# mandt-lab/vbq

Measured on AMD Instinct MI355X. Metric: quantized latents/sec (32-lambda sweep; one count per (element, lambda) pair and entropy-model build), higher is better.
Workload: dtype f32; 1 GPU; kodak24_c256 [36864 x 256] f32, 32-lambda sweep, N=10; step = two-pass entropy-model build (quantizer.py:82-150); elements_per_gpu=9437184, lambdas=32, parallelism=element-sharded x1, launch=one HIP graph replay per step

## Files before the change

### include/vbq.h

```cpp
#ifndef VBQ_H_
#define VBQ_H_

#include <stddef.h>
#include <stdint.h>

#ifdef __cplusplus
extern "C" {
#endif

#define VBQ_ABI_VERSION 5

enum {
    VBQ_OK = 0,
    VBQ_ERR_INVALID_ARGUMENT = -1,
    VBQ_ERR_UNSUPPORTED = -2,
    VBQ_ERR_LAUNCH = -3,
    VBQ_ERR_WORKSPACE = -4
};

enum {
    VBQ_LAYOUT_BC = 0,
    VBQ_LAYOUT_CB = 1,
    VBQ_LAYOUT_BC_TO_CB = 2
};
// ... 3 lines not shown
    VBQ_MODE_F64_SCORE = 1
};

int vbq_abi_version(void);
const char *vbq_last_error(void);


enum { VBQ_GRID_K1 = 0, VBQ_GRID_K1T = 1 };
int vbq_solve_grid(int32_t kernel, int64_t n_rows, int32_t n_ch, int32_t workgroups_per_cu, int32_t reserved_workgroups,
                   int64_t *h_grid);

int vbq_device_count(void);
int vbq_device_name(int dev, char *buf, size_t buflen);

size_t vbq_quantize_workspace_bytes(int32_t n_ch, int32_t n_lambda, int32_t N);

int vbq_check_inputs_f32(const float *d_mu, const float *d_sigma, int64_t n, uint32_t *d_bad, void *stream);

int vbq_quantize_f32(const float *d_mu, const float *d_sigma, int64_t n_rows, int32_t n_ch,
                     int32_t layout, const float *d_table_lm, const float *d_level_len,
                     const double *h_lambdas, int32_t n_lambda, int32_t N, int32_t mode,
                     uint16_t *d_out_idx, float *d_out_zhat, float *d_out_bits,
                     void *d_workspace, size_t workspace_bytes, void *stream);

int vbq_n_bit_intervals_f32(const float *d_z_cb, int64_t n_rows, int32_t n_ch, const float *d_table_lm, int32_t N,
                            float *d_left, float *d_right, void *stream);

int vbq_quantize_rows_f32(const float *d_mu, const float *d_sigma, int64_t n_rows, int32_t n_ch,
                          int32_t layout, const float *d_table_lm, const float *d_level_len,
                          const double *h_lambdas, int32_t n_lambda, int32_t N, int32_t mode,
                          uint16_t *d_out_idx, float *d_out_zhat, float *d_out_bits,
                          void *d_workspace, size_t workspace_bytes, int64_t row_begin, int64_t row_end,
                          int32_t workgroups_per_cu, int32_t reserved_workgroups, void *stream);

int vbq_level_counts_f32(const float *d_mu, const float *d_sigma, int64_t n_rows, int32_t n_ch,
                         int32_t layout, const float *d_table_lm, const float *d_level_len,
                         const double *h_lambdas, int32_t n_lambda, int32_t N, int64_t *d_level_counts,
                         void *d_workspace, size_t workspace_bytes, int32_t reserved_workgroups, void *stream);

int vbq_code_lengths_from_counts(const void *d_counts, int32_t counts_are_i32, int64_t n,
                                 const float *d_lut, int64_t lut_n, int32_t level_period,
                                 float *d_out_len, float *d_out_model, void *stream);

typedef void (*vbq_f32_loop)(char **args, const intptr_t *dimensions, const intptr_t *steps, void *data);
typedef struct vbq_host_stage {
    const void *h_counts;
    int32_t counts_are_i32;
    int32_t add_level;
    int64_t n_rows;
    int64_t K;
    float add_n_smoothing;
    int32_t status;
    vbq_f32_loop log2_loop;
    void *log2_data;
    float *h_out_model;
    float *h_out_len;
    int64_t runs;
} vbq_host_stage;
int vbq_host_neg_log2_freq_f32(const void *h_counts, int32_t counts_are_i32, int64_t n_rows, int64_t K, float add_n_smoothing,
                               int32_t add_level, vbq_f32_loop log2_loop, void *log2_data, float *h_out_model,
                               float *h_out_len);
void vbq_host_stage_run(void *stage);

int vbq_argmax_candidates_f32(const float *d_P, const float *d_len, int32_t len_per_lambda,
                              const float *d_mu, const float *d_sigma, int64_t n_elems,
                              const double *h_lambdas, int32_t n_lambda, int32_t M, int32_t mode,
// ... 163 lines not shown
```

### vbq_amd/_lib.py

```python
from __future__ import annotations

import ctypes as C
import os


_LIB = None

c_f32p = C.c_void_p
c_u16p = C.c_void_p

OK = 0
ABI_VERSION = 5
LAYOUT_BC, LAYOUT_CB, LAYOUT_BC_TO_CB = 0, 1, 2
MODE_F32, MODE_F64_SCORE = 0, 1
BMSHJ_PARAMS_PER_CHANNEL = 43
COMM_ID_BYTES = 128

SIGNATURES = {
    "vbq_abi_version": (C.c_int, []),
    "vbq_last_error": (C.c_char_p, []),
    "vbq_solve_grid": (C.c_int, [C.c_int32, C.c_int64, C.c_int32, C.c_int32, C.c_int32, C.POINTER(C.c_int64)]),
    "vbq_device_count": (C.c_int, []),
    "vbq_device_name": (C.c_int, [C.c_int, C.c_char_p, C.c_size_t]),
    "vbq_quantize_workspace_bytes": (C.c_size_t, [C.c_int32, C.c_int32, C.c_int32]),
    "vbq_check_inputs_f32": (C.c_int, [C.c_void_p, C.c_void_p, C.c_int64, C.c_void_p, C.c_void_p]),
    "vbq_quantize_f32": (C.c_int, [C.c_void_p, C.c_void_p, C.c_int64, C.c_int32, C.c_int32, C.c_void_p, C.c_void_p,
                                   C.POINTER(C.c_double), C.c_int32, C.c_int32, C.c_int32, C.c_void_p, C.c_void_p,
                                   C.c_void_p, C.c_void_p, C.c_size_t, C.c_void_p]),
    "vbq_n_bit_intervals_f32": (C.c_int, [C.c_void_p, C.c_int64, C.c_int32, C.c_void_p, C.c_int32, C.c_void_p, C.c_void_p,
                                          C.c_void_p]),
    "vbq_quantize_rows_f32": (C.c_int, [C.c_void_p, C.c_void_p, C.c_int64, C.c_int32, C.c_int32, C.c_void_p, C.c_void_p,
                                        C.POINTER(C.c_double), C.c_int32, C.c_int32, C.c_int32, C.c_void_p, C.c_void_p,
                                        C.c_void_p, C.c_void_p, C.c_size_t, C.c_int64, C.c_int64, C.c_int32, C.c_int32, C.c_void_p]),
    "vbq_level_counts_f32": (C.c_int, [C.c_void_p, C.c_void_p, C.c_int64, C.c_int32, C.c_int32, C.c_void_p, C.c_void_p,
                                       C.POINTER(C.c_double), C.c_int32, C.c_int32, C.c_void_p, C.c_void_p, C.c_size_t,
                                       C.c_int32, C.c_void_p]),
    "vbq_code_lengths_from_counts": (C.c_int, [C.c_void_p, C.c_int32, C.c_int64, C.c_void_p, C.c_int64, C.c_int32,
                                               C.c_void_p, C.c_void_p, C.c_void_p]),
    "vbq_host_neg_log2_freq_f32": (C.c_int, [C.c_void_p, C.c_int32, C.c_int64, C.c_int64, C.c_float, C.c_int32, C.c_void_p, C.c_void_p,
                                             C.c_void_p, C.c_void_p]),
    "vbq_host_stage_run": (None, [C.c_void_p]),
    "vbq_histogram_rows_u16": (C.c_int, [C.c_void_p, C.c_int64, C.c_int32, C.c_int32, C.c_int32, C.c_int32, C.c_void_p,
                                         C.c_int32, C.c_int64, C.c_int64, C.c_void_p]),
    "vbq_xi_intervals_f64": (C.c_int, [C.c_void_p, C.c_int64, C.c_int32, C.c_void_p, C.c_void_p, C.c_void_p]),
    "vbq_xi_select_f64": (C.c_int, [C.c_void_p, C.c_void_p, C.c_void_p, C.c_int64, C.c_int32, C.c_double, C.c_void_p,
                                    C.c_void_p, C.c_void_p, C.c_void_p, C.c_void_p]),
    "vbq_quantize_notebook_f64": (C.c_int, [C.c_void_p, C.c_void_p, C.c_int64, C.c_void_p, C.POINTER(C.c_double),
                                            C.c_int32, C.c_int32, C.c_void_p, C.c_void_p, C.c_void_p]),
    "vbq_histogram_u16": (C.c_int, [C.c_void_p, C.c_int64, C.c_int32, C.c_int32, C.c_int32, C.c_int32, C.c_void_p,
                                    C.c_void_p]),
    "vbq_histogram_u16_i32": (C.c_int, [C.c_void_p, C.c_int64, C.c_int32, C.c_int32, C.c_int32, C.c_int32,
                                        C.c_void_p, C.c_void_p]),
    "vbq_histogram_models_u16": (C.c_int, [C.c_void_p, C.c_int64, C.c_int32, C.c_int32, C.c_int32, C.c_void_p, C.c_int32,
                                           C.c_void_p, C.c_int64, C.c_void_p, C.c_void_p]),
    "vbq_index_max_u16": (C.c_int, [C.c_void_p, C.c_int64, C.c_void_p, C.c_void_p]),
    "vbq_moments_f32": (C.c_int, [C.c_void_p, C.c_int64, C.c_int32, C.c_int32, C.c_void_p, C.c_void_p]),
    "vbq_numpy_sum_sq_workspace_bytes": (C.c_size_t, [C.c_int64]),
    "vbq_numpy_sum_sq_f32": (C.c_int, [C.c_void_p, C.c_int64, C.c_void_p, C.c_void_p, C.c_size_t, C.c_void_p]),
    "vbq_numpy_row_sums_workspace_bytes": (C.c_size_t, [C.c_int64, C.c_int64]),
    "vbq_numpy_row_sums_f32": (C.c_int, [C.c_void_p, C.c_int64, C.c_int64, C.c_void_p, C.c_void_p, C.c_size_t, C.c_void_p]),
    "vbq_gather_f32": (C.c_int, [C.c_void_p, C.c_int64, C.c_int32, C.c_int32, C.c_int32, C.c_int32, C.c_void_p,
                                 C.c_int32, C.c_void_p, C.c_int32, C.c_void_p]),
    "vbq_rd_sums_u16": (C.c_int, [C.c_void_p, C.c_void_p, C.c_void_p, C.c_int64, C.c_int32, C.c_int32, C.c_int32, C.c_int32,
                                  C.c_void_p, C.c_void_p, C.c_int32, C.c_void_p, C.c_void_p]),
    "vbq_transpose_f32": (C.c_int, [C.c_void_p, C.c_int64, C.c_int64, C.c_void_p, C.c_void_p]),
    "vbq_transpose_planes": (C.c_int, [C.c_void_p, C.c_int64, C.c_int64, C.c_int64, C.c_int32, C.c_void_p, C.c_void_p]),
# ... 121 lines not shown
```

### vbq_amd/csrc/vbq_latents.hip

```cpp
#include <atomic>

#include <type_traits>

#include "vbq_common.h"

namespace vbq {
namespace {

__global__ void __launch_bounds__(256)
k_prep_planes(const float *__restrict__ in0, const float *__restrict__ in1, long rows, long cols, float *__restrict__ out0,
              float *__restrict__ out1, int sqrt1, int v4) {
    __shared__ float tile[64][65];
    const bool second = blockIdx.y == 1;
    const float *in = second ? in1 : in0;
    float *out = second ? out1 : out0;
    const int kind = second ? sqrt1 : 0;
    auto f = [kind](float x) { return kind == 0 ? x : sqrtf(kind == 2 ? expf(x) : x); };
    const long ctiles = (cols + 63) / 64;
    const long r0 = ((long)blockIdx.x / ctiles) * 64, c0 = ((long)blockIdx.x % ctiles) * 64;
    if (v4 && r0 + 64 <= rows && c0 + 64 <= cols) {
        float4 v[4];
#pragma unroll
        for (int k = 0; k < 4; ++k) {
            const int i = threadIdx.x + 256 * k, lr = i >> 4, lc = (i & 15) * 4;
// ... 441 lines not shown
    VBQ_REQUIRE(d_lut_levels && n_lut_levels > n_rows && d_level_counts && d_level_len && d_raw_models && d_counts,
                VBQ_ERR_INVALID_ARGUMENT, "vbq_build_entropy_models_f32: null pointer argument, or a code-length table shorter than n_rows + 1");
    VBQ_REQUIRE((d_models == nullptr) == (d_lut_ranks == nullptr) && (!d_lut_ranks || n_lut_ranks > n_rows), VBQ_ERR_INVALID_ARGUMENT,
                "vbq_build_entropy_models_f32: d_models and d_lut_ranks go together (n_rows + 1 entries)");
    const size_t need = vbq_build_entropy_models_workspace_bytes(n_rows, n_ch, n_lambda, N);
    VBQ_REQUIRE(d_workspace && workspace_bytes >= need, VBQ_ERR_WORKSPACE,
                "vbq_build_entropy_models_f32: workspace of %zu bytes given, %zu needed", workspace_bytes, need);
    VBQ_REQUIRE((reinterpret_cast<uintptr_t>(d_workspace) & 255) == 0, VBQ_ERR_INVALID_ARGUMENT,
                "vbq_build_entropy_models_f32: workspace must be 256-byte aligned");
    const size_t E = (size_t)n_rows * (size_t)n_ch;
    const int64_t N1 = N + 1;
    char *w = static_cast<char *>(d_workspace);
    float *mu_cb = reinterpret_cast<float *>(w);
    w += align256(E * sizeof(float));
    float *sg_cb = reinterpret_cast<float *>(w);
    w += align256(E * sizeof(float));
    uint16_t *idx = reinterpret_cast<uint16_t *>(w);
    w += align256((size_t)n_lambda * E * sizeof(uint16_t));
    const size_t qws = vbq_quantize_workspace_bytes(n_ch, n_lambda, N);
    hipStream_t st = reinterpret_cast<hipStream_t>(stream);
    int rc = vbq_prep_planes_f32(d_means_bc, d_spread_bc, spread_kind, n_rows, n_ch, mu_cb, sg_cb, stream);
    if (rc != VBQ_OK) return rc;
    hipError_t e = hipMemsetAsync(d_level_counts, 0, sizeof(int64_t) * (size_t)n_lambda * (size_t)n_ch * (size_t)N1, st);
    if (e != hipSuccess) {
        set_error("vbq_build_entropy_models_f32: hipMemsetAsync: %s", hipGetErrorString(e));
        return VBQ_ERR_LAUNCH;
    }
    rc = vbq_level_counts_f32(mu_cb, sg_cb, n_rows, n_ch, VBQ_LAYOUT_CB, d_table_lm, nullptr, h_lambdas, n_lambda, N, d_level_counts, w, qws,
                              reserved_workgroups, stream);
    if (rc != VBQ_OK) return rc;
    rc = vbq_code_lengths_from_counts(d_level_counts, 0, (int64_t)n_lambda * n_ch * N1, d_lut_levels, n_lut_levels, (int32_t)N1, d_level_len,
                                      d_raw_models, stream);
    if (rc != VBQ_OK) return rc;
    rc = vbq_quantize_rows_f32(mu_cb, sg_cb, n_rows, n_ch, VBQ_LAYOUT_CB, d_table_lm, d_level_len, h_lambdas, n_lambda, N, VBQ_MODE_F32, idx,
                               nullptr, nullptr, w, qws, 0, n_rows, 0, reserved_workgroups, stream);
    if (rc != VBQ_OK) return rc;
    return vbq_histogram_models_u16(idx, n_rows, n_ch, n_lambda, N, d_counts, counts_are_i32, d_lut_ranks, n_lut_ranks, d_models, stream);
}
```

### vbq_amd/csrc/vbq_quantize_fast.hip

```cpp
#include <string.h>

#include "vbq_common.h"

namespace vbq {
namespace {

constexpr int kFastThreads = 256;
#ifndef VBQ_FAST_NE
#define VBQ_FAST_NE 2
#endif
#ifndef VBQ_FAST_WAVES
#define VBQ_FAST_WAVES 4
#endif
#ifndef VBQ_SLOW_INLINE
#define VBQ_SLOW_INLINE __noinline__
#endif
constexpr int kFastNE = VBQ_FAST_NE;

__device__ __forceinline__ float dist_cost(float P, float mu, double rinv) {
    const float d = __fsub_rn(P, mu);
    const float t = (float)__dmul_rn((double)d, rinv);
    const float q = __fmul_rn(t, t);
    return __fmul_rn(0.5f, q);
}
// ... 73 lines not shown
        const float po = tb[off + jo];
        const float dj = dist_cost(pj, z, sg);
        const float dn = dist_cost(po, z, sg);
        const bool j_is_left = below && !swap;
        r.dL = j_is_left ? dj : dn;
        r.dR = j_is_left ? dn : dj;
        r.posL = j_is_left ? j : (uint32_t)jo;
        r.posR = j_is_left ? (uint32_t)jo : j;
    }
    g = 2 * g + (below ? 1u : 0u);
    return r;
}

template <int N>
__device__ VBQ_SLOW_INLINE uint32_t exact_rank_scan(const float *tb, float z, float sigma, const float *pen) {
    const double sg = __ddiv_rn(1.0, (double)sigma);
    uint32_t g = 0;
    float bestL = 0.f, bestR = 0.f;
    uint32_t rkL = 0, rkR = 0;
    for (int n = 0; n <= N; ++n) {
        const LevelInfo<N> li = descend<N>(tb, n, z, sg, g);
        const float p = pen[n];
        const float cL = __fadd_rn(li.dL, p);
        if (n == 0 || cL < bestL) { bestL = cL; rkL = ((2 * li.posL + 1) << (N - n)) - 1; }
        if (n >= 1) {
            const float cR = __fadd_rn(li.dR, p);
            if (n == 1 || cR < bestR) { bestR = cR; rkR = ((2 * li.posR + 1) << (N - n)) - 1; }
        }
    }
    if (N == 0) return rkL;
    return (bestL <= bestR) ? rkL : rkR;
}

template <int N, int MODE>
__global__ void __launch_bounds__(kFastThreads, VBQ_FAST_WAVES)
k_quant_fast(const float *__restrict__ mu, const float *__restrict__ sg, long n_per_ch, long ch_stride, int C,
             const float *__restrict__ table, Lambdas32 lam, const float *__restrict__ len,
             int L, uint16_t *__restrict__ out_idx, float *__restrict__ out_zhat,
             float *__restrict__ out_bits, long E, int vec_ok, int dbg,
             unsigned long long *__restrict__ level_counts) {
    constexpr int T = table_size(N);
    constexpr int N1 = N + 1;
    constexpr int NE = kFastNE;
    constexpr bool EXTRA = MODE == 1;
    constexpr bool COUNT = MODE == 2;
    const bool never_flag = dbg == 2;
    constexpr int PS = (N1 + 3) & ~3;
    __shared__ float tb[T + 1];
    __shared__ uint32_t scratch[N1 * NE * kFastThreads];
    __shared__ __align__(16) float penl[kMaxLambdaChunk * PS];
    const int c = blockIdx.y;
    if (COUNT) {
        for (int i = threadIdx.x; i < N1 * NE * kFastThreads; i += blockDim.x) scratch[i] = 0;
    }
    for (int i = threadIdx.x; i < T; i += blockDim.x) tb[i] = table[(long)c * T + i];
    int odd = 0;
    for (int i = threadIdx.x; i < L * PS; i += blockDim.x) {
        const int l = i / PS, n = i - l * PS;
        const float p = n < N1 ? __fmul_rn(lam.lam[l], len ? len[((long)l * C + c) * N1 + n] : (float)n) : 0.0f;
        penl[i] = p;
        odd |= (len != nullptr && !(p == 0.0f || (p >= 1.8189894e-12f && p <= 1.1805916e21f))) ? 1 : 0;
    }
    const bool force_slow = dbg == 1 || __syncthreads_or(odd) != 0;

    const long base = (long)c * ch_stride;
    const long nquads = (n_per_ch + NE - 1) / NE;

    auto load_group = [&](long q, float (&m)[NE], float (&sv)[NE]) {
        const long i0 = q * NE;
        if (!(vec_ok & 2) && (vec_ok & 1) && (i0 + NE <= n_per_ch)) {
            if constexpr (NE == 4) {
                const float4 mv = *reinterpret_cast<const float4 *>(mu + base + i0);
                const float4 s4v = *reinterpret_cast<const float4 *>(sg + base + i0);
                m[0] = mv.x; m[1] = mv.y; m[2] = mv.z; m[3] = mv.w;
                sv[0] = s4v.x; sv[1] = s4v.y; sv[2] = s4v.z; sv[3] = s4v.w;
            } else {
                const float2 mv = *reinterpret_cast<const float2 *>(mu + base + i0);
                const float2 s2v = *reinterpret_cast<const float2 *>(sg + base + i0);
// ... 120 lines not shown
                            lvl[k] = (uint32_t)N - (uint32_t)__builtin_ctz(exact_rank_scan<N>(tb, m4[k], s4[k], pp) + 1u);
                }
                const uint32_t lane = threadIdx.x & 63u;
                const uint32_t inc = (lane & 16u) ? 0x10000u : 1u;
#pragma unroll
                for (int k = 0; k < NE; ++k)
                    if (i0 + k < n_per_ch) atomicAdd(&scratch[((uint32_t)(l * N1) + lvl[k]) * 16u + (lane & 15u)], inc);
                continue;
            }
            uint32_t pk[NE];
#pragma unroll
            for (int k = 0; k < NE; ++k) {
                const int n1 = __builtin_ctz(~ne[k]);
                pk[k] = scratch[(n1 * NE + k) * kFastThreads + threadIdx.x];
            }
            uint64_t fm[NE];
#pragma unroll
            for (int k = 0; k < NE; ++k) {
                const uint64_t multi = __builtin_amdgcn_uicmp((uint32_t)__popc(ne[k]), (uint32_t)N, 33);
                const uint32_t thr = __float_as_uint(__fmul_rn(S[k], 1.9073486328125e-06f));
                const uint64_t lr_close = __builtin_amdgcn_uicmp(pk[k], thr, 37);
                rank[k] = pk[k] & ((2u << N) - 1u);
                fm[k] = never_flag ? 0ull : (force_slow ? ~0ull : (multi | lr_close));
            }
            uint64_t any_flag = 0;
#pragma unroll
            for (int k = 0; k < NE; ++k) any_flag |= fm[k];
            if (any_flag != 0) {
                const uint32_t lane = __lane_id();
#pragma unroll
                for (int k = 0; k < NE; ++k)
                    if ((fm[k] >> lane) & 1ull) rank[k] = exact_rank_scan<N>(tb, m4[k], s4[k], pp);
            }
            const long o = (long)l * E + base + i0;
            float zh[NE], bt[NE];
            if (EXTRA) {
#pragma unroll
                for (int k = 0; k < NE; ++k) {
                    const uint32_t kk = rank[k] + 1;
                    const int tz = __builtin_ctz(kk);
                    const int lvl = N - tz;
                    const uint32_t pos = kk >> (tz + 1);
                    zh[k] = tb[(1 << lvl) - 1 + pos];
                    bt[k] = len ? len[((long)l * C + c) * N1 + lvl] : (float)lvl;
                }
            }
            if (full) {
                if constexpr (NE == 4) {
                    uint2 pk2;
                    pk2.x = rank[0] | (rank[1] << 16);
                    pk2.y = rank[2] | (rank[3] << 16);
                    *reinterpret_cast<uint2 *>(out_idx + o) = pk2;
                    if (EXTRA) {
                        if (out_zhat) *reinterpret_cast<float4 *>(out_zhat + o) = make_float4(zh[0], zh[1], zh[2], zh[3]);
                        if (out_bits) *reinterpret_cast<float4 *>(out_bits + o) = make_float4(bt[0], bt[1], bt[2], bt[3]);
                    }
                } else {
                    store_idx2<false>(reinterpret_cast<uint32_t *>(out_idx + o), rank[0] | (rank[1] << 16));
                    if (EXTRA) {
                        if (out_zhat) *reinterpret_cast<float2 *>(out_zhat + o) = make_float2(zh[0], zh[1]);
                        if (out_bits) *reinterpret_cast<float2 *>(out_bits + o) = make_float2(bt[0], bt[1]);
                    }
                }
            } else {
#pragma unroll
                for (int k = 0; k < NE; ++k) {
                    if (i0 + k < n_per_ch) {
                        out_idx[o + k] = (uint16_t)rank[k];
                        if (EXTRA) {
                            if (out_zhat) out_zhat[o + k] = zh[k];
                            if (out_bits) out_bits[o + k] = bt[k];
                        }
                    }
                }
            }
        }
    }
    if constexpr (COUNT) {
        __syncthreads();
        for (int i = threadIdx.x; i < L * N1; i += blockDim.x) {
            unsigned int v = 0;
#pragma unroll
            for (int j = 0; j < 16; ++j) {
                const unsigned int w = scratch[i * 16 + j];
                v += (w & 0xffffu) + (w >> 16);
            }
            const int l = i / N1, n = i - l * N1;
            if (v) atomicAdd(&level_counts[((long)l * C + c) * N1 + n], (unsigned long long)v);
        }
    }
}


#ifndef VBQ_HULL_WAVES
#define VBQ_HULL_WAVES 4
#endif
#ifndef VBQ_HULL_NE
#define VBQ_HULL_NE 2
#endif
#ifndef VBQ_HULL_THREADS
#define VBQ_HULL_THREADS 256
#endif
constexpr int kHullThreads = VBQ_HULL_THREADS;
#ifndef VBQ_HULL_COPIES
#define VBQ_HULL_COPIES 16
#endif
constexpr int kHullKeys = 2048;
// ... 831 lines not shown
        }
        constexpr int64_t max_iters = 65000 / ((64 / 32) * (kFastThreads / 64) * kFastNE);
        if (counting && (iters + gx - 1) / gx > max_iters) gx = (iters + max_iters - 1) / max_iters;
    }
    if (gx < 1) gx = 1;
    *out_gx = gx;
    *out_resident = resident;
}

template <int N>
int launch_quant_fast(const float *mu, const float *sg, int64_t n_per_ch, int64_t ch_stride, int32_t n_ch, const float *table,
                      const Lambdas32 &lam, const float *len, int32_t L, uint16_t *out_idx, float *out_zhat,
                      float *out_bits, int64_t E, int vec_ok,
                      unsigned long long *level_counts, int wg_per_cu, int reserved, hipStream_t st) {
    int64_t gx = 1;
    bool resident = false;
    quant_fast_grid(n_per_ch, n_ch, wg_per_cu, reserved, level_counts != nullptr, &gx, &resident);
    if (resident) vec_ok |= 4;
    const dim3 grid((unsigned)gx, (unsigned)n_ch), block(kFastThreads);
    const int dbg = fast_debug();
    if (level_counts)
        hipLaunchKernelGGL((k_quant_fast<N, 2>), grid, block, 0, st, mu, sg, (long)n_per_ch, (long)ch_stride, (int)n_ch, table,
                           lam, len, (int)L, out_idx, out_zhat, out_bits, (long)E, vec_ok, dbg, level_counts);
    else if (out_zhat || out_bits)
        hipLaunchKernelGGL((k_quant_fast<N, 1>), grid, block, 0, st, mu, sg, (long)n_per_ch, (long)ch_stride, (int)n_ch, table,
                           lam, len, (int)L, out_idx, out_zhat, out_bits, (long)E, vec_ok, dbg, level_counts);
    else
        hipLaunchKernelGGL((k_quant_fast<N, 0>), grid, block, 0, st, mu, sg, (long)n_per_ch, (long)ch_stride, (int)n_ch, table,
                           lam, len, (int)L, out_idx, out_zhat, out_bits, (long)E, vec_ok, dbg, level_counts);
    VBQ_CHECK_LAUNCH("quant_fast");
    return VBQ_OK;
}

template <int N>
int launch_quant_pruned(const float *mu, const float *sg, int64_t n_per_ch, int64_t ch_stride, int32_t n_ch, const float *table,
                        const Lambdas32 &lam, const float *len, int32_t L, uint16_t *out_idx, int64_t E, int vec_ok, hipStream_t st) {
    if (L < 1 || L > kPrunedMaxL) return 1;
    const int64_t npairs = (n_per_ch + 1) / 2;
    int64_t gx = (npairs + 255) / 256;
    int64_t cap = (int64_t)num_cus() * 4 / n_ch;
    if (cap < 1) cap = 1;
    if (gx > cap) gx = cap;
    const int dbg = fast_debug();
    const dim3 grid((unsigned)gx, (unsigned)n_ch), block(256);
#define VBQ_PRUNED_CASE(LLv)                                                                                          \
    case LLv:                                                                                                          \
        hipLaunchKernelGGL((k_quant_pruned<N, LLv>), grid, block, 0, st, mu, sg, (long)n_per_ch, (long)ch_stride, (int)n_ch, \
                           table, lam, len, out_idx, (long)E, vec_ok, dbg);                                            \
        break;
    switch (L) {
        VBQ_PRUNED_CASE(1) VBQ_PRUNED_CASE(2) VBQ_PRUNED_CASE(3) VBQ_PRUNED_CASE(4)
        default: return 1;
    }
#undef VBQ_PRUNED_CASE
    VBQ_CHECK_LAUNCH("quant_pruned");
    return VBQ_OK;
}


static bool build_hull_sweep(const double *lam, int L, HullSweep &sw) {
    if (L < 1 || L > 32) return false;
    int order[32];
    for (int i = 0; i < L; ++i) order[i] = i;
    for (int i = 1; i < L; ++i)
        for (int j = i; j > 0 && (float)lam[order[j]] < (float)lam[order[j - 1]]; --j) { const int t = order[j]; order[j] = order[j - 1]; order[j - 1] = t; }
    int prev_key = -1;
// ... 96 lines not shown
                                       const Lambdas32 &, const float *, int32_t, uint16_t *, float *, float *, int64_t, \
                                       int, unsigned long long *, int, int, hipStream_t);
VBQ_FOR_EACH_N(VBQ_INST_FAST)
#undef VBQ_INST_FAST
#define VBQ_INST_PRUNED(NN)                                                                                           \
    template int launch_quant_pruned<NN>(const float *, const float *, int64_t, int64_t, int32_t, const float *,     \
                                         const Lambdas32 &, const float *, int32_t, uint16_t *, int64_t, int, hipStream_t);
VBQ_FOR_EACH_N(VBQ_INST_PRUNED)
#undef VBQ_INST_PRUNED

}

extern "C" int vbq_solve_grid(int32_t kernel, int64_t n_rows, int32_t n_ch, int32_t workgroups_per_cu, int32_t reserved_workgroups,
                              int64_t *h_grid) {
    using namespace vbq;
    VBQ_REQUIRE(h_grid && n_rows >= 1 && n_ch >= 1 && n_ch <= 65535, VBQ_ERR_INVALID_ARGUMENT, "vbq_solve_grid: bad sizes or null pointer");
    VBQ_REQUIRE(kernel == VBQ_GRID_K1 || kernel == VBQ_GRID_K1T, VBQ_ERR_INVALID_ARGUMENT, "vbq_solve_grid: unknown kernel %d", kernel);
    VBQ_REQUIRE(workgroups_per_cu >= 0 && workgroups_per_cu <= 5, VBQ_ERR_INVALID_ARGUMENT, "vbq_solve_grid: workgroups_per_cu=%d not in 0..5",
                workgroups_per_cu);
    const int reserved = reserved_workgroups < 0 ? 0 : reserved_workgroups;
    if (kernel == VBQ_GRID_K1) {
        int64_t gx = 1;
        bool resident = false;
        quant_fast_grid(n_rows, n_ch, workgroups_per_cu, reserved, false, &gx, &resident);
        h_grid[0] = gx;
        h_grid[2] = resident ? 1 : 0;
    } else {
        h_grid[0] = level_counts_hull_grid(n_rows, n_ch, reserved);
        h_grid[2] = 1;
    }
    h_grid[1] = n_ch;
    return VBQ_OK;
}
```

### vbq_amd/ops.py

```python
from __future__ import annotations

import ctypes as C
from typing import Optional, Sequence

import numpy as np
import torch

from . import _lib
from ._lib import LAYOUT_BC, LAYOUT_BC_TO_CB, LAYOUT_CB, MODE_F32, MODE_F64_SCORE, VBQError, check
from .tables import table_size

_LAYOUTS = {"bc": LAYOUT_BC, "cb": LAYOUT_CB, LAYOUT_BC: LAYOUT_BC, LAYOUT_CB: LAYOUT_CB}
_MODES = {"f32": MODE_F32, "f64": MODE_F64_SCORE, MODE_F32: MODE_F32, MODE_F64_SCORE: MODE_F64_SCORE}


_raw_stream = getattr(torch._C, "_cuda_getCurrentRawStream", None)


def raw_stream(device: torch.device) -> int:
    if _raw_stream is not None:
        return _raw_stream(device.index if device.index is not None else torch.cuda.current_device())
    return torch.cuda.current_stream(device).cuda_stream


# ... 110 lines not shown
    mu, sigma, rows, Cc, table_lm, L, level_len = _solve_inputs(mu, sigma, table_lm, lambdas, N, level_len, layout)
    h = _lib.lib()
    if to_planes and mu.dim() == 2 and Cc > 1:
        layout, oshape = LAYOUT_BC_TO_CB, (L, Cc, rows)
    else:
        oshape = (L,) + tuple(mu.shape)
    idx = _out(out_idx, oshape, torch.uint16, mu.device, "out_idx")
    zhat = _out(out_zhat, oshape, torch.float32, mu.device, "out_zhat", want_zhat)
    bits = _out(out_bits, oshape, torch.float32, mu.device, "out_bits", want_bits)
    want_zhat, want_bits = zhat is not None, bits is not None
    wsb = h.vbq_quantize_workspace_bytes(Cc, L, N)
    ws = _workspace(workspace, wsb, mu.device)
    if mu.numel() == 0:
        out = (idx,) + ((zhat,) if want_zhat else ()) + ((bits,) if want_bits else ())
        return out if len(out) > 1 else idx
    if rows_range is None and not workgroups_per_cu and reserved_workgroups is None:
        check(h.vbq_quantize_f32(_ptr(mu), _ptr(sigma), rows, Cc, layout, _ptr(table_lm), _ptr(level_len),
                                 _doubles(lambdas), L, N, mode, _ptr(idx), _ptr(zhat), _ptr(bits), _ptr(ws), wsb,
                                 _stream(mu)), "vbq_quantize_f32")
    else:
        r0, r1 = (0, rows) if rows_range is None else (int(rows_range[0]), int(rows_range[1]))
        check(h.vbq_quantize_rows_f32(_ptr(mu), _ptr(sigma), rows, Cc, layout, _ptr(table_lm), _ptr(level_len),
                                      _doubles(lambdas), L, N, mode, _ptr(idx), _ptr(zhat), _ptr(bits), _ptr(ws), wsb,
                                      r0, r1, int(workgroups_per_cu), -1 if reserved_workgroups is None else int(reserved_workgroups),
                                      _stream(mu)), "vbq_quantize_rows_f32")
    out = (idx,)
    if want_zhat:
        out += (zhat,)
    if want_bits:
        out += (bits,)
    return out if len(out) > 1 else idx


def check_inputs(mu: torch.Tensor, sigma: torch.Tensor):
    mu, sigma = _pair(mu, sigma)
    bad = torch.zeros(2, dtype=torch.uint32, device=mu.device)
    check(_lib.lib().vbq_check_inputs_f32(_ptr(mu), _ptr(sigma), mu.numel(), _ptr(bad), _stream(mu)), "vbq_check_inputs_f32")
    b = bad.cpu().numpy()
    if b[0] or b[1]:
        raise ValueError(f"invalid latents: {int(b[0])} non-finite means, {int(b[1])} standard deviations that are not finite and positive")


def level_counts(mu: torch.Tensor, sigma: torch.Tensor, table_lm: torch.Tensor, lambdas: Sequence[float], *,
                 N: int = 10, level_len: Optional[torch.Tensor] = None, layout="bc", out: Optional[torch.Tensor] = None,
                 workspace: Optional[torch.Tensor] = None, reserved_workgroups: Optional[int] = None):
    to_planes = layout in ("bc->cb", LAYOUT_BC_TO_CB)
    layout = LAYOUT_BC if to_planes else _LAYOUTS[layout]
    mu, sigma, rows, Cc, table_lm, L, level_len = _solve_inputs(mu, sigma, table_lm, lambdas, N, level_len, layout)
    if to_planes and mu.dim() == 2 and Cc > 1:
        layout = LAYOUT_BC_TO_CB
    if out is None:
        out = torch.zeros((L, Cc, N + 1), dtype=torch.int64, device=mu.device)
    else:
        _out(out, (L, Cc, N + 1), torch.int64, mu.device, "out")
    h = _lib.lib()
    wsb = h.vbq_quantize_workspace_bytes(Cc, L, N)
    ws = _workspace(workspace, wsb, mu.device)
    if mu.numel():
        check(h.vbq_level_counts_f32(_ptr(mu), _ptr(sigma), rows, Cc, layout, _ptr(table_lm), _ptr(level_len),
                                     _doubles(lambdas), L, N, _ptr(out), _ptr(ws), wsb,
                                     -1 if reserved_workgroups is None else int(reserved_workgroups), _stream(mu)),
              "vbq_level_counts_f32")
    return out


def code_lengths_from_counts(counts: torch.Tensor, lut: torch.Tensor, *, level_period: int = 0, want_len: bool = True,
# ... 437 lines not shown
```

### vbq_amd/pipeline.py

```python
from __future__ import annotations

from typing import Optional, Sequence

import numpy as np
import torch

import ctypes as _C
import glob as _glob
import os as _os

from . import entropy as _entropy
from . import ops
from ._lib import VBQError

_HIP = None


def _hip_runtime():
    global _HIP
    if _HIP is None:
        cands = _glob.glob(_os.path.join(_os.path.dirname(torch.__file__), "lib", "libamdhip64.so*")) + ["libamdhip64.so"]
        for c in cands:
            try:
                _HIP = _C.CDLL(c)
# ... 213 lines not shown
        self.host_stage_kind = None
        self._len_stage = None
        if self.lut1 is None:
            self._len_stage = NativeHostStage(self.level_counts, self.raw_models, self.level_len, add_n_smoothing, loop) if loop else \
                HostStage([self.level_counts], [self.level_len, self.raw_models], lengths_host)
            self.host_stage_kind = "native" if loop else "python"
        self._model_stages = None
        if self.lut2 is None and self.models is not None:
            self._model_stages = [NativeHostStage(c, self.models, None, add_n_smoothing, loop) if loop else
                                  HostStage([c], [self.models], lambda counts: _entropy.neg_log2_freq(counts, smooth))
                                  for c in self._counts2]
            self.host_stage_kind = "native" if loop else "python"
        if n_chunks is None:
            n_chunks = 1
        self.chunks = chunk_bounds(self.rows, n_chunks)
        self.k1_workgroups_per_cu = 3
        self.side = torch.cuda.Stream(device=self.dev) if len(self.chunks) > 1 else None
        self._events = [torch.cuda.Event() for _ in self.chunks] if self.side is not None else []
        self.reducers = [None, None]
        self.works = [None, None]
        self._models_pending = [False, False]
        self.timers = None
        self.collectives = True
        if self.world > 1 and counts_dtype == torch.int32:
            from .dist import CountsAllReduce
            self.reducers = [CountsAllReduce(L * C * T, self.dev, max_global_count=self.global_rows, group=group) for _ in range(2)]
        if reserved_workgroups is None:
            payload = 0
            if self.world > 1:
                r = self.reducers[0]
                payload = r.payload_bytes(self.counts) if r is not None else self.counts.numel() * self.counts.element_size()
            reserved_workgroups = 64 if payload >= (4 << 20) else 0
        self.reserved_workgroups = int(reserved_workgroups)

    @property
    def idx(self) -> torch.Tensor:
        if self._idx is None:
            L, C = self.L, self.C
            self._idx = self._kept(("idx", L, C, self.rows, str(self.dev)),
                                   lambda: torch.empty((L, C, self.rows), dtype=torch.uint16, device=self.dev))
        return self._idx

    @property
    def one_call_ok(self) -> bool:
        return (self.world == 1 and self.side is None and self.lut1 is not None and
                (self.models is None or self.lut2 is not None) and self.timers is None)

    def run_one_call(self, means_bc: torch.Tensor, spread_bc: torch.Tensor, spread: str = "sigma"):
        if not self.one_call_ok:
            raise VBQError("run_one_call: this build needs the staged form (sharded, chunked, timed, or a -log2 step that is not tabulated)")
        means_bc = ops._dev(means_bc, torch.float32, "means")
        spread_bc = ops._dev(spread_bc, torch.float32, "spread")
        if tuple(means_bc.shape) != (self.rows, self.C) or means_bc.shape != spread_bc.shape:
            raise ValueError(f"expected two [{self.rows}, {self.C}] tensors, got {tuple(means_bc.shape)} / {tuple(spread_bc.shape)}")
        h = ops._lib.lib()
        wsb = h.vbq_build_entropy_models_workspace_bytes(self.rows, self.C, self.L, self.N)
        ws = self._kept(("ws_build", self.L, self.C, self.rows, self.N, str(self.dev)),
                        lambda: torch.empty(max(wsb, 256), dtype=torch.uint8, device=self.dev))
        fused = self.models is not None
        ops._lib.check(h.vbq_build_entropy_models_f32(
            ops._ptr(means_bc), ops._ptr(spread_bc), ops._spread_kind(spread), self.rows, self.C, ops._ptr(self.table),
            ops._doubles(self.lambdas), self.L, self.N, ops._ptr(self.lut1), self.lut1.numel(),
            ops._ptr(self.lut2) if fused else None, self.lut2.numel() if fused else 0, ops._ptr(self.level_counts),
            ops._ptr(self.level_len), ops._ptr(self.raw_models), ops._ptr(self.counts), int(self.counts.dtype == torch.int32),
            ops._ptr(self.models) if fused else None, ops._ptr(ws), ws.numel(), self._reserved(), ops._stream(means_bc)),
            "vbq_build_entropy_models_f32")
# ... 4 lines not shown
        return self.reserved_workgroups if self.collectives else 0

    def pass1(self, mu_cb, sg_cb, level_len=None):
        self.level_counts.zero_()
        self._t("k1h", 0)
        ops.level_counts(mu_cb, sg_cb, self.table, self.lambdas, N=self.N, level_len=level_len, layout="cb",
                         out=self.level_counts, workspace=self.ws, reserved_workgroups=self._reserved())
        self._t("k1h", 1)
        if self.world > 1 and self.collectives:
            torch.distributed.all_reduce(self.level_counts, group=self.level_group)
        return self.level_counts

    def _t(self, name, phase):
        if self.timers is not None:
            self.timers(name, phase)

    def lengths(self):
        if self.lut1 is not None:
            ops.code_lengths_from_counts(self.level_counts, self.lut1, level_period=self.N + 1, out_len=self.level_len,
                                         out_model=self.raw_models)
        else:
            self._len_stage.enqueue()
        return self.level_len, self.raw_models

    def pass2(self, mu_cb, sg_cb, level_len):
        if self.world > 1:
            self._slot ^= 1
            self.counts = self._counts2[self._slot]
        self.wait(self._slot)
        main = torch.cuda.current_stream(self.dev)
        self._models_current = False
        if self.side is None and self.world == 1:
            fused = self.lut2 is not None and self.models is not None
            self._t("k1", 0)
            ops.quantize(mu_cb, sg_cb, self.table, self.lambdas, N=self.N, level_len=level_len, layout="cb",
                         out_idx=self.idx, workspace=self.ws, reserved_workgroups=self._reserved())
            self._t("k1", 1)
            self._t("k2", 0)
            ops.histogram_models(self.idx, self.C, self.counts, N=self.N, lut=self.lut2 if fused else None,
                                 models=self.models if fused else None)
            self._t("k2", 1)
            self._models_current = fused
            return self.idx, self.counts
        self.counts.zero_()
        if self.side is None:
            self._t("k1", 0)
            ops.quantize(mu_cb, sg_cb, self.table, self.lambdas, N=self.N, level_len=level_len, layout="cb",
                         out_idx=self.idx, workspace=self.ws, reserved_workgroups=self._reserved())
            self._t("k1", 1)
            self._t("k2", 0)
            ops.histogram(self.idx, self.C, N=self.N, layout="cb", out=self.counts)
            self._t("k2", 1)
        else:
            self.side.wait_stream(main)
            for j, (r0, r1) in enumerate(self.chunks):
                self._t("k1", 0)
                ops.quantize(mu_cb, sg_cb, self.table, self.lambdas, N=self.N, level_len=level_len, layout="cb",
                             out_idx=self.idx, workspace=self.ws, rows=(r0, r1), workgroups_per_cu=self.k1_workgroups_per_cu,
                             reserved_workgroups=self._reserved())
                self._t("k1", 1)
                self._events[j].record(main)
                with torch.cuda.stream(self.side):
                    self.side.wait_event(self._events[j])
                    self._t("k2", 0)
                    ops.histogram(self.idx, self.C, N=self.N, layout="cb", out=self.counts, rows=(r0, r1))
                    self._t("k2", 1)
            main.wait_stream(self.side)
        if self.world > 1 and self.collectives:
            if self.reducers[self._slot] is not None:
                self.works[self._slot] = self.reducers[self._slot].start(self.counts)
            else:
                self.works[self._slot] = torch.distributed.all_reduce(self.counts, group=self.group, async_op=True)
        return self.idx, self.counts
# ... 87 lines not shown
```

Baseline: 476.0 billion latents/s.

## Fuse rank counting into quantize kernel for the last lambdas via shared window

Adds a new quantize kernel mode that counts ranks directly while quantizing, for up to the last 16 lambdas. It uses an LDS window histogram for the common shallow ranks and global atomics for the rest. The separate histogram pass then runs only on the remaining lambdas, with code lengths computed from the fused counts. The goal is to cut the idx re-read and histogram kernel cost, at the price of more atomics and LDS pressure inside the quantize kernel.

```diff
diff --git a/include/vbq.h b/include/vbq.h
--- a/include/vbq.h
+++ b/include/vbq.h
@@ -59,6 +59,12 @@
                           uint16_t *d_out_idx, float *d_out_zhat, float *d_out_bits,
                           void *d_workspace, size_t workspace_bytes, int64_t row_begin, int64_t row_end,
                           int32_t workgroups_per_cu, int32_t reserved_workgroups, void *stream);
+
+int32_t vbq_count_split(const double *h_lambdas, int32_t n_lambda, int32_t N, int32_t counts_are_i32);
+int vbq_quantize_count_f32(const float *d_mu_cb, const float *d_sigma_cb, int64_t n_rows, int32_t n_ch,
+                           const float *d_table_lm, const float *d_level_len, const double *h_lambdas,
+                           int32_t n_lambda, int32_t N, uint16_t *d_out_idx, int32_t l_split, int32_t *d_counts,
+                           int32_t reserved_workgroups, void *stream);
 
 int vbq_level_counts_f32(const float *d_mu, const float *d_sigma, int64_t n_rows, int32_t n_ch,
                          int32_t layout, const float *d_table_lm, const float *d_level_len,
diff --git a/vbq_amd/_lib.py b/vbq_amd/_lib.py
--- a/vbq_amd/_lib.py
+++ b/vbq_amd/_lib.py
@@ -32,6 +32,10 @@
     "vbq_quantize_rows_f32": (C.c_int, [C.c_void_p, C.c_void_p, C.c_int64, C.c_int32, C.c_int32, C.c_void_p, C.c_void_p,
                                         C.POINTER(C.c_double), C.c_int32, C.c_int32, C.c_int32, C.c_void_p, C.c_void_p,
                                         C.c_void_p, C.c_void_p, C.c_size_t, C.c_int64, C.c_int64, C.c_int32, C.c_int32, C.c_void_p]),
+    "vbq_count_split": (C.c_int32, [C.POINTER(C.c_double), C.c_int32, C.c_int32, C.c_int32]),
+    "vbq_quantize_count_f32": (C.c_int, [C.c_void_p, C.c_void_p, C.c_int64, C.c_int32, C.c_void_p, C.c_void_p,
+                                         C.POINTER(C.c_double), C.c_int32, C.c_int32, C.c_void_p, C.c_int32, C.c_void_p,
+                                         C.c_int32, C.c_void_p]),
     "vbq_level_counts_f32": (C.c_int, [C.c_void_p, C.c_void_p, C.c_int64, C.c_int32, C.c_int32, C.c_void_p, C.c_void_p,
                                        C.POINTER(C.c_double), C.c_int32, C.c_int32, C.c_void_p, C.c_void_p, C.c_size_t,
                                        C.c_int32, C.c_void_p]),
diff --git a/vbq_amd/csrc/vbq_latents.hip b/vbq_amd/csrc/vbq_latents.hip
--- a/vbq_amd/csrc/vbq_latents.hip
+++ b/vbq_amd/csrc/vbq_latents.hip
@@ -497,8 +497,22 @@
     rc = vbq_code_lengths_from_counts(d_level_counts, 0, (int64_t)n_lambda * n_ch * N1, d_lut_levels, n_lut_levels, (int32_t)N1, d_level_len,
                                       d_raw_models, stream);
     if (rc != VBQ_OK) return rc;
-    rc = vbq_quantize_rows_f32(mu_cb, sg_cb, n_rows, n_ch, VBQ_LAYOUT_CB, d_table_lm, d_level_len, h_lambdas, n_lambda, N, VBQ_MODE_F32, idx,
-                               nullptr, nullptr, w, qws, 0, n_rows, 0, reserved_workgroups, stream);
+    const int32_t l_split = vbq_count_split(h_lambdas, n_lambda, N, counts_are_i32);
+    if (l_split >= n_lambda) {
+        rc = vbq_quantize_rows_f32(mu_cb, sg_cb, n_rows, n_ch, VBQ_LAYOUT_CB, d_table_lm, d_level_len, h_lambdas, n_lambda, N, VBQ_MODE_F32,
+                                   idx, nullptr, nullptr, w, qws, 0, n_rows, 0, reserved_workgroups, stream);
+        if (rc != VBQ_OK) return rc;
+        return vbq_histogram_models_u16(idx, n_rows, n_ch, n_lambda, N, d_counts, counts_are_i32, d_lut_ranks, n_lut_ranks, d_models, stream);
+    }
+    rc = vbq_quantize_count_f32(mu_cb, sg_cb, n_rows, n_ch, d_table_lm, d_level_len, h_lambdas, n_lambda, N, idx, l_split,
+                                static_cast<int32_t *>(d_counts), reserved_workgroups, stream);
     if (rc != VBQ_OK) return rc;
-    return vbq_histogram_models_u16(idx, n_rows, n_ch, n_lambda, N, d_counts, counts_are_i32, d_lut_ranks, n_lut_ranks, d_models, stream);
-}
+    if (l_split > 0) {
+        rc = vbq_histogram_models_u16(idx, n_rows, n_ch, l_split, N, d_counts, counts_are_i32, d_lut_ranks, n_lut_ranks, d_models, stream);
+        if (rc != VBQ_OK) return rc;
+    }
+    if (!d_models) return VBQ_OK;
+    const int64_t done = (int64_t)l_split * n_ch * table_size(N);
+    return vbq_code_lengths_from_counts(static_cast<int32_t *>(d_counts) + done, 1, (int64_t)(n_lambda - l_split) * n_ch * table_size(N),
+                                        d_lut_ranks, n_lut_ranks, 0, nullptr, d_models + done, stream);
+}
diff --git a/vbq_amd/csrc/vbq_quantize_fast.hip b/vbq_amd/csrc/vbq_quantize_fast.hip
--- a/vbq_amd/csrc/vbq_quantize_fast.hip
+++ b/vbq_amd/csrc/vbq_quantize_fast.hip
@@ -129,6 +129,8 @@
     return (bestL <= bestR) ? rkL : rkR;
 }
 
+constexpr int kWinRows = 16;
+constexpr int kWinBins = 128;
 template <int N, int MODE>
 __global__ void __launch_bounds__(kFastThreads, VBQ_FAST_WAVES)
 k_quant_fast(const float *__restrict__ mu, const float *__restrict__ sg, long n_per_ch, long ch_stride, int C,
@@ -141,6 +143,20 @@
     constexpr int NE = kFastNE;
     constexpr bool EXTRA = MODE == 1;
     constexpr bool COUNT = MODE == 2;
+    constexpr bool WIN = MODE == 3;
+    static_assert(!WIN || N == 10, "the window numbers the shallow ranks of N = 10");
+    int l_split = 0, l_win0 = 0;
+    uint32_t *win = nullptr;
+    uint32_t *rank_counts = nullptr;
+    if constexpr (WIN) {
+        __shared__ uint32_t win_s[kWinRows * kWinBins];
+        win = win_s;
+        rank_counts = reinterpret_cast<uint32_t *>(level_counts);
+        l_split = dbg >> 8;
+        dbg &= 0xff;
+        l_win0 = l_split > L - kWinRows ? l_split : L - kWinRows;
+        for (int i = threadIdx.x; i < kWinRows * kWinBins; i += blockDim.x) win[i] = 0;
+    }
     const bool never_flag = dbg == 2;
     constexpr int PS = (N1 + 3) & ~3;
     __shared__ float tb[T + 1];
@@ -327,6 +343,38 @@
                 for (int k = 0; k < NE; ++k)
                     if ((fm[k] >> lane) & 1ull) rank[k] = exact_rank_scan<N>(tb, m4[k], s4[k], pp);
             }
+            if constexpr (WIN) {
+                if (l >= l_split) {
+                    uint32_t *crow = rank_counts + ((long)l * C + c) * T;
+                    const int wr = l - l_win0;
+                    if (wr >= 0) {
+                        uint32_t *wrow = win + wr * kWinBins;
+                        uint32_t q1[NE];
+                        uint32_t n0 = 0;
+                        bool rest[NE];
+#pragma unroll
+                        for (int k = 0; k < NE; ++k) {
+                            q1[k] = rank[k] + 1u;
+                            const bool valid = i0 + k < n_per_ch;
+                            const bool lvl0 = q1[k] == (1u << N);
+                            n0 += (uint32_t)__popcll(__builtin_amdgcn_ballot_w64(valid && lvl0));
+                            rest[k] = valid && !lvl0;
+                        }
+                        if (n0 != 0u && (threadIdx.x & 63u) == 0u) atomicAdd(&wrow[(kWinBins / 2) ^ (kWinBins / 32)], n0);
+#pragma unroll
+                        for (int k = 0; k < NE; ++k) {
+                            if (rest[k]) {
+                                if ((q1[k] & 15u) == 0u) atomicAdd(&wrow[(q1[k] >> 4) ^ (q1[k] >> 8)], 1u);
+                                else atomicAdd(&crow[rank[k]], 1u);
+                            }
+                        }
+                    } else {
+#pragma unroll
+                        for (int k = 0; k < NE; ++k)
+                            if (i0 + k < n_per_ch) atomicAdd(&crow[rank[k]], 1u);
+                    }
+                }
+            }
             const long o = (long)l * E + base + i0;
             float zh[NE], bt[NE];
             if (EXTRA) {
@@ -368,6 +416,17 @@
                         }
                     }
                 }
+            }
+        }
+    }
+    if constexpr (WIN) {
+        __syncthreads();
+        for (int i = threadIdx.x; i < (L - l_win0) * kWinBins; i += blockDim.x) {
+            const uint32_t v = win[i];
+            if (v) {
+                const uint32_t sl = (uint32_t)i & (kWinBins - 1);
+                const uint32_t w = sl ^ (sl >> 4);
+                atomicAdd(&rank_counts[((long)(l_win0 + i / kWinBins) * C + c) * T + 16u * w - 1u], v);
             }
         }
     }
@@ -1265,6 +1324,21 @@
     return VBQ_OK;
 }
 
+int launch_quant_fast_count10(const float *mu, const float *sg, int64_t n_per_ch, int64_t ch_stride, int32_t n_ch, const float *table,
+                              const Lambdas32 &lam, const float *len, int32_t L, uint16_t *out_idx, int64_t E, int vec_ok,
+                              int32_t l_split, uint32_t *counts, int reserved, hipStream_t st) {
+    int64_t gx = 1;
+    bool resident = false;
+    quant_fast_grid(n_per_ch, n_ch, 0, reserved, false, &gx, &resident);
+    if (resident) vec_ok |= 4;
+    const int dbg = fast_debug() | ((int)l_split << 8);
+    hipLaunchKernelGGL((k_quant_fast<10, 3>), dim3((unsigned)gx, (unsigned)n_ch), dim3(kFastThreads), 0, st, mu, sg, (long)n_per_ch,
+                       (long)ch_stride, (int)n_ch, table, lam, len, (int)L, out_idx, (float *)nullptr, (float *)nullptr, (long)E,
+                       vec_ok, dbg, reinterpret_cast<unsigned long long *>(counts));
+    VBQ_CHECK_LAUNCH("quant_fast_count");
+    return VBQ_OK;
+}
+
 template <int N>
 int launch_quant_pruned(const float *mu, const float *sg, int64_t n_per_ch, int64_t ch_stride, int32_t n_ch, const float *table,
                         const Lambdas32 &lam, const float *len, int32_t L, uint16_t *out_idx, int64_t E, int vec_ok, hipStream_t st) {
@@ -1427,3 +1501,57 @@
     h_grid[1] = n_ch;
     return VBQ_OK;
 }
+
+namespace vbq {
+constexpr double kCountSplitLambda = __builtin_huge_val();
+}
+extern "C" int32_t vbq_count_split(const double *h_lambdas, int32_t n_lambda, int32_t N, int32_t counts_are_i32) {
+    using namespace vbq;
+    if (!h_lambdas || n_lambda < 1 || n_lambda > kMaxLambdaChunk || N != 10 || !counts_are_i32) return n_lambda < 0 ? 0 : n_lambda;
+    for (int i = 0; i < n_lambda; ++i) {
+        if (!(h_lambdas[i] >= 1.9e-12 && h_lambdas[i] <= 1.8e19)) return n_lambda;
+        if (i > 0 && !(h_lambdas[i] > h_lambdas[i - 1])) return n_lambda;
+    }
+    int32_t split = n_lambda;
+    while (split > 0 && h_lambdas[split - 1] >= kCountSplitLambda) --split;
+    return split < n_lambda - kWinRows ? n_lambda - kWinRows : split;
+}
+
+extern "C" int vbq_quantize_count_f32(const float *d_mu_cb, const float *d_sigma_cb, int64_t n_rows, int32_t n_ch,
+                                      const float *d_table_lm, const float *d_level_len, const double *h_lambdas,
+                                      int32_t n_lambda, int32_t N, uint16_t *d_out_idx, int32_t l_split, int32_t *d_counts,
+                                      int32_t reserved_workgroups, void *stream) {
+    using namespace vbq;
+    VBQ_REQUIRE(n_rows >= 1 && n_rows <= 0x7fffffffLL && n_ch >= 1 && n_ch <= 65535 && n_lambda >= 1, VBQ_ERR_INVALID_ARGUMENT,
+                "vbq_quantize_count_f32: bad sizes n_rows=%lld n_ch=%d n_lambda=%d", (long long)n_rows, n_ch, n_lambda);
+    VBQ_REQUIRE(d_mu_cb && d_sigma_cb && d_table_lm && h_lambdas && d_out_idx && d_counts, VBQ_ERR_INVALID_ARGUMENT,
+                "vbq_quantize_count_f32: null pointer argument");
+    VBQ_REQUIRE(l_split >= 0 && l_split <= n_lambda, VBQ_ERR_INVALID_ARGUMENT, "vbq_quantize_count_f32: l_split=%d not in 0..%d",
+                l_split, n_lambda);
+    VBQ_REQUIRE(N == 10 && n_lambda <= kMaxLambdaChunk, VBQ_ERR_UNSUPPORTED,
+                "vbq_quantize_count_f32: built for N = 10 and at most %d lambdas (use vbq_quantize_f32 + vbq_histogram_models_u16)",
+                kMaxLambdaChunk);
+    Lambdas32 l32;
+    for (int i = 0; i < kMaxLambdaChunk; ++i) {
+        VBQ_REQUIRE(i >= n_lambda || (h_lambdas[i] >= 1.9e-12 && h_lambdas[i] <= 1.8e19), VBQ_ERR_UNSUPPORTED,
+                    "vbq_quantize_count_f32: lambda %d outside the fast kernel's range [1.9e-12, 1.8e19]", i);
+        l32.lam[i] = i < n_lambda ? (float)h_lambdas[i] : 0.0f;
+    }
+    hipStream_t st = reinterpret_cast<hipStream_t>(stream);
+    constexpr int64_t T = table_size(10);
+    const int64_t E = n_rows * (int64_t)n_ch;
+    if (l_split < n_lambda &&
+        hipMemsetAsync(d_counts + (int64_t)l_split * n_ch * T, 0, sizeof(int32_t) * (size_t)(n_lambda - l_split) * (size_t)n_ch * (size_t)T,
+                       st) != hipSuccess) {
+        set_error("vbq_quantize_count_f32: hipMemsetAsync failed");
+        return VBQ_ERR_LAUNCH;
+    }
+    const int vec_ok = ((reinterpret_cast<uintptr_t>(d_mu_cb) | reinterpret_cast<uintptr_t>(d_sigma_cb)) % 4 == 0) &&
+                       (reinterpret_cast<uintptr_t>(d_out_idx) % 2 == 0);
+    const int reserved = reserved_workgroups < 0 ? 0 : reserved_workgroups;
+    if (l_split == n_lambda)
+        return launch_quant_fast<10>(d_mu_cb, d_sigma_cb, n_rows, n_rows, n_ch, d_table_lm, l32, d_level_len, n_lambda, d_out_idx, nullptr,
+                                     nullptr, E, vec_ok, nullptr, 0, reserved, st);
+    return launch_quant_fast_count10(d_mu_cb, d_sigma_cb, n_rows, n_rows, n_ch, d_table_lm, l32, d_level_len, n_lambda, d_out_idx, E,
+                                     vec_ok, l_split, reinterpret_cast<uint32_t *>(d_counts), reserved, st);
+}
diff --git a/vbq_amd/ops.py b/vbq_amd/ops.py
--- a/vbq_amd/ops.py
+++ b/vbq_amd/ops.py
@@ -166,6 +166,29 @@
     return out if len(out) > 1 else idx
 
 
+def count_split(lambdas: Sequence[float], *, N: int = 10, counts_dtype=torch.int32) -> int:
+    return int(_lib.lib().vbq_count_split(_doubles(lambdas), len(lambdas), int(N), int(counts_dtype == torch.int32)))
+
+
+def quantize_count(mu: torch.Tensor, sigma: torch.Tensor, table_lm: torch.Tensor, lambdas: Sequence[float], l_split: int,
+                   counts: torch.Tensor, *, level_len: Optional[torch.Tensor] = None, out_idx: Optional[torch.Tensor] = None,
+                   reserved_workgroups: Optional[int] = None):
+    N = 10
+    mu, sigma, rows, Cc, table_lm, L, level_len = _solve_inputs(mu, sigma, table_lm, lambdas, N, level_len, LAYOUT_CB)
+    idx = _out(out_idx, (L,) + tuple(mu.shape), torch.uint16, mu.device, "out_idx")
+    _out(counts, (L, Cc, table_size(N)), torch.int32, mu.device, "counts")
+    if not 0 <= int(l_split) <= L:
+        raise ValueError(f"l_split={l_split} not in 0..{L}")
+    if mu.numel() == 0:
+        counts[int(l_split):].zero_()
+        return idx
+    check(_lib.lib().vbq_quantize_count_f32(_ptr(mu), _ptr(sigma), rows, Cc, _ptr(table_lm), _ptr(level_len), _doubles(lambdas), L, N,
+                                            _ptr(idx), int(l_split), _ptr(counts),
+                                            -1 if reserved_workgroups is None else int(reserved_workgroups), _stream(mu)),
+          "vbq_quantize_count_f32")
+    return idx
+
+
 def check_inputs(mu: torch.Tensor, sigma: torch.Tensor):
     mu, sigma = _pair(mu, sigma)
     bad = torch.zeros(2, dtype=torch.uint32, device=mu.device)
diff --git a/vbq_amd/pipeline.py b/vbq_amd/pipeline.py
--- a/vbq_amd/pipeline.py
+++ b/vbq_amd/pipeline.py
@@ -269,6 +269,9 @@
                 payload = r.payload_bytes(self.counts) if r is not None else self.counts.numel() * self.counts.element_size()
             reserved_workgroups = 64 if payload >= (4 << 20) else 0
         self.reserved_workgroups = int(reserved_workgroups)
+        self.l_split = self.L
+        if self.world == 1 and self.side is None:
+            self.l_split = ops.count_split(self.lambdas, N=self.N, counts_dtype=counts_dtype)
 
     @property
     def idx(self) -> torch.Tensor:
@@ -339,13 +342,21 @@
         self._models_current = False
         if self.side is None and self.world == 1:
             fused = self.lut2 is not None and self.models is not None
+            ls = self.l_split
             self._t("k1", 0)
-            ops.quantize(mu_cb, sg_cb, self.table, self.lambdas, N=self.N, level_len=level_len, layout="cb",
-                         out_idx=self.idx, workspace=self.ws, reserved_workgroups=self._reserved())
+            if ls < self.L:
+                ops.quantize_count(mu_cb, sg_cb, self.table, self.lambdas, ls, self.counts, level_len=level_len,
+                                   out_idx=self.idx, reserved_workgroups=self._reserved())
+            else:
+                ops.quantize(mu_cb, sg_cb, self.table, self.lambdas, N=self.N, level_len=level_len, layout="cb",
+                             out_idx=self.idx, workspace=self.ws, reserved_workgroups=self._reserved())
             self._t("k1", 1)
             self._t("k2", 0)
-            ops.histogram_models(self.idx, self.C, self.counts, N=self.N, lut=self.lut2 if fused else None,
-                                 models=self.models if fused else None)
+            if ls > 0:
+                ops.histogram_models(self.idx[:ls], self.C, self.counts[:ls], N=self.N, lut=self.lut2 if fused else None,
+                                     models=self.models[:ls] if fused else None)
+            if ls < self.L and fused:
+                ops.code_lengths_from_counts(self.counts[ls:], self.lut2, want_len=False, out_model=self.models[ls:])
             self._t("k2", 1)
             self._models_current = fused
             return self.idx, self.counts
```

New measurement: 468.0 billion latents/s. -1.7%, worse.
